# hidasib/GRU4Rec

Measured on AMD Instinct MI355X. Metric: mini-batches/sec (gru4rec.py:661), RSC15-shaped batch=128 n_sample=2048 BPR-max, higher is better.
Workload: dtype f32

## Files before the change

gru4rec_amd/csrc/g4r_device.cuh:

```cuda
#pragma once
#include <hip/hip_runtime.h>
#include <stdint.h>

#include "../../include/gru4rec_hip.h"

typedef float f32x4 __attribute__((ext_vector_type(4)));

#define G4R_EPS_LOSS 1e-24f
#define G4R_EPS_ADAGRAD 1e-6f

#if defined(G4R_MUTATE) && G4R_MUTATE == 1
#define G4R_MUT_ACC(x) ((x) * 1.01f)
#else
#define G4R_MUT_ACC(x) (x)
#endif
#if defined(G4R_MUTATE) && G4R_MUTATE == 2
#define G4R_MUT_STEP(x) ((x) * 1.01f)
#else
#define G4R_MUT_STEP(x) (x)
#endif
#if defined(G4R_MUTATE) && G4R_MUTATE == 3
#define G4R_MUT_DACC(x) ((x) * 1.01f)
#else
#define G4R_MUT_DACC(x) (x)
#endif

#if defined(G4R_MUTATE) && G4R_MUTATE == 6
#define G4R_MUT_ROW(n, x) ((n) == 0 ? (x) * 1.5f : (x))
#else
#define G4R_MUT_ROW(n, x) (x)
#endif
#if defined(G4R_MUTATE) && G4R_MUTATE == 5
#define G4R_MUT_XSCALE(x) ((x) * 1.01f)
#else
#define G4R_MUT_XSCALE(x) (x)
#endif

#define G4R_STREAM_SAMPLE 0x53414D50u
#define G4R_STREAM_DROP_EMBED 0x44454D42u
#define G4R_STREAM_DROP_HIDDEN 0x44484944u
#define G4R_STREAM_TIEBREAK 0x54494542u

#if defined(__HIP_DEVICE_COMPILE__)
#define GAS __attribute__((address_space(1)))
#else
#define GAS
#endif
#define GP(T) GAS T*

__device__ __forceinline__ float4 ld4(const GAS float* p) { return *(const GAS float4*)p; }
__device__ __forceinline__ void st4(GAS float* p, float4 v) { *(GAS float4*)p = v; }
__device__ __forceinline__ int4 ldi4(const GAS int* p) { return *(const GAS int4*)p; }
#if defined(__HIP_DEVICE_COMPILE__)
// ... 60 lines not shown
    GP(const int) in_idx; GP(const int) out_idx; GP(const int) Mplan;
    GP(const unsigned char) reset;
    GP(const int) ST;
    int gl;
    GP(const float) lq_tgt; GP(const float) lq_smp;
    GP(StepState) st;
    GP(long long) dbgclk;
    GP(const float) zrow;
    GP(long long) dbgtile;
    GP(float) xbase;
    long long xstride;
    int xn, xoffSx, xoffSy, xoffSBy;
    int xmode, xoffDg;
    GP(float) dyp;
    int bbn[G4R_MAX_LAYERS];
    GP(float) vp;
    int defer_mask, dRcap;
    long long dSx_stride, dSy_stride, dSBy_stride;
    GP(int) last_use;
    GP(int) dcand;
    GP(int) dlist;
    GP(unsigned) dstat;
    GP(float) drp;
};
#define G4R_SLOT(m, g) ((size_t)((g) & (long long)(m).defer_mask))
#define G4R_DSX(m, g) ((m).dSx + G4R_SLOT(m, g) * (size_t)(m).dSx_stride)
#define G4R_DSY(m, g) ((m).dSy + G4R_SLOT(m, g) * (size_t)(m).dSy_stride)
#define G4R_DSBY(m, g) ((m).dSBy + G4R_SLOT(m, g) * (size_t)(m).dSBy_stride)

#if defined(G4R_CLK_TRACE)
#define G4R_DBGCLK(m) ((m).dbgclk)
#define G4R_DBGTILE(m) ((m).dbgtile)
#else
#define G4R_DBGCLK(m) ((GAS long long*)nullptr)
#define G4R_DBGTILE(m) ((GAS long long*)nullptr)
#endif
#define G4R_TICK(m, kern, phase)                                                                     \
    do {                                                                                             \
        if (G4R_DBGCLK(m) && blockIdx.x == 0 && blockIdx.y == 0 && threadIdx.x == 0)                  \
            G4R_DBGCLK(m)[(kern) * 16 + (phase)] = wall_clock64();                                       \
    } while (0)

template <int CTRL>
__device__ __forceinline__ float dpp_mov(float v) {
    return __builtin_bit_cast(float, __builtin_amdgcn_update_dpp(0, __builtin_bit_cast(int, v), CTRL, 0xF, 0xF, true));
}
// ... 138 lines not shown
```

gru4rec_amd/csrc/g4r_host_create.hpp:

```cpp

int g4r_device_count(void) {
    int n = 0;
    if (hipGetDeviceCount(&n) != hipSuccess) return 0;
    return n;
}
const char* g4r_last_error(void) { return g_err.c_str(); }
#ifndef G4R_HIPCC_VERSION
#define G4R_HIPCC_VERSION "unknown"
#endif
const char* g4r_version(void) { return "gru4rec_hip 0.4 (gfx950; hipcc " G4R_HIPCC_VERSION "; isa-audited)"; }
int g4r_sizeof_config(void) { return (int)sizeof(g4r_config); }

static int build_lean_args(g4r_model* m) {
    DevModel& d = m->dm;
    const StepKernels& k = m->kern;
    const int L = d.n_layers;
    std::vector<LeanV> av(L); std::vector<LeanH> ah(L); std::vector<LeanDa> aa(L); std::vector<LeanDy> ay(L);
    const bool constrained = d.embed_mode == G4R_EMBED_CONSTRAINED;
    bool any_layer = false;
    for (int l = 0; l < L; ++l) {
        if (k.fwd[l] != FWD_LEAN) continue;
        any_layer = true;
        LeanV& v = av[l]; memset(&v, 0, sizeof(v));
        v.Wx = d.dense_p + d.offWx[l]; v.Wrz = d.dense_p + d.offWrz[l]; v.Bh = d.dense_p + d.offBh[l];
// ... 33 lines not shown
        q.col_item = d.col_item; q.occ_idx = d.occ_idx + d.B; q.occ_fl = d.occ_fl; q.mp = nullptr; q.dbg = d.dbgclk; q.dbgtile = d.dbgtile; q.R = d.R; q.pub_fl = d.xmode == 0 ? 1 : 0; q.logq = d.logq;
        m->h_leanS = q;
        if (dalloc(m, &m->d_leanS, (size_t)1)) return -1;
    }
    if (k.score_bwd == SB_LEAN) {
        LeanB q; memset(&q, 0, sizeof(q));
        q.accBy = d.accBy; q.occ_fl = d.occ_fl; q.dSy = d.dSy; q.dAy = d.dAy; q.dSBy = d.dSBy; q.dABy = d.dABy; q.dhpart = d.dhpart; q.dbg = d.dbgclk; q.dbgtile = d.dbgtile;
        q.dSy_stride = d.dSy_stride; q.dSBy_stride = d.dSBy_stride; q.defer_mask = d.defer_mask; q.generic = d.generic;
        q.ndh = cdiv(d.Dtop + 1, 64); q.nA = cdiv(d.ldSc, 16) * q.ndh; q.nrb = cdiv(d.B, 16); q.ndb = cdiv(d.Dtop, 64); q.lr = d.lr;
        m->h_leanB = q;
        if (dalloc(m, &m->d_leanB, (size_t)1)) return -1;
        HIPCHK(hipMemcpyAsync(m->d_leanB, &m->h_leanB, sizeof(LeanB), hipMemcpyHostToDevice, m->stream));
    }
    if (k.update == UP_LEAN) {
        LeanU u; memset(&u, 0, sizeof(u));
        u.mp = nullptr; u.st = d.st; u.Wy = d.Wy; u.E = d.E; u.accWy = d.accWy; u.accE = d.accE; u.velWy = d.velWy; u.velE = d.velE;
        u.By = d.By; u.accBy = d.accBy; u.velBy = d.velBy; u.dAx = d.dAx; u.dAy = d.dAy; u.dABy = d.dABy;
        u.dense_p = d.dense_p; u.dense_acc = d.dense_acc; u.dense_vel = d.dense_vel; u.yin0 = d.yin0; u.meta = d.cur_in + 2 * d.B;
        u.dbg = d.dbgclk; u.dbgtile = d.dbgtile; u.n_items = d.n_items; u.constrained = constrained ? 1 : 0; u.wE = d.Ein; u.wY = d.Dtop;
        u.lr = d.lr; u.mom = d.mom; u.lmbd = d.lmbd;
        m->h_leanU = u;
        const std::vector<DenseTile> tiles = dense_tiles(d, 16, 64);
        m->ntiles16 = (int)tiles.size();
        if (dalloc(m, &m->d_tiles16, tiles.size()) || dalloc(m, &m->d_leanU, (size_t)1)) return -1;
        HIPCHK(hipMemcpyAsync(m->d_tiles16, tiles.data(), tiles.size() * sizeof(DenseTile), hipMemcpyHostToDevice, m->stream));
        HIPCHK(hipStreamSynchronize(m->stream));
    }
    HIPCHK(hipStreamSynchronize(m->stream));
    return 0;
}

static KernelSwitches read_switches(const g4r_config& cfg) {
    KernelSwitches w;
    w.no_lean = getenv("G4R_NO_LEAN") != nullptr; w.no_mt = getenv("G4R_NO_MT") != nullptr; w.no_bmt = getenv("G4R_NO_BMT") != nullptr;
    w.no_merge = getenv("G4R_NO_MERGE") != nullptr;
    w.allow_lean_update = env_int("G4R_LEAN_UPDATE", 1) != 0; w.defer = env_int("G4R_DEFER", cfg.defer_updates) != 0;
    w.p2_geo = env_int("G4R_P2_GEO", -1); w.ba_geo = env_int("G4R_BA_GEO", -1);
    w.wide2 = env_int("G4R_WIDE2", -1); w.p1_ks = env_int("G4R_P1_KS", 128); w.bb_ks = env_int("G4R_BB_KS", 0);
    const char* skip = getenv("G4R_SKIP_KN");
    w.skip_kn = skip ? strtoull(skip, nullptr, 0) : 0ull;
    return w;
}

int g4r_create(const g4r_config* cfg, g4r_model** out) {
    if (!cfg || !out) return fail("null argument");
    if (cfg->n_layers < 1 || cfg->n_layers > G4R_MAX_LAYERS) return fail("n_layers out of range");
    if (cfg->batch_size < 1 || cfg->n_items < 1) return fail("batch_size / n_items must be positive");
    for (int l = 0; l < cfg->n_layers; ++l)
        if (cfg->layers[l] % 4 != 0 || cfg->layers[l] < 4 || cfg->layers[l] > 1024)
            return fail("layer sizes must be multiples of 4 in [4, 1024]");
    if (cfg->embed_mode == G4R_EMBED_SEPARATE && (cfg->embedding % 4 != 0 || cfg->embedding < 4 || cfg->embedding > 1024))
        return fail("embedding must be a multiple of 4 in [4, 1024]");
    if (cfg->embed_mode != G4R_EMBED_CONSTRAINED && cfg->embed_mode != G4R_EMBED_SEPARATE && cfg->embed_mode != G4R_EMBED_ONEHOT)
        return fail("unsupported embedding mode");
    if (cfg->embed_mode == G4R_EMBED_ONEHOT && 3 * cfg->layers[0] > 1024)
        return fail("one-hot input: 3 * layers[0] must be <= 1024 (row width of the Wx[0] table)");
    if (cfg->loss < 0 || cfg->loss > G4R_LOSS_XE_LOGIT) return fail("unsupported loss");
    if (cfg->smoothing != 0.f && cfg->loss != G4R_LOSS_XE && cfg->loss != G4R_LOSS_XE_LOGIT) return fail("smoothing needs a cross-entropy loss");
// ... 251 lines not shown
```

gru4rec_amd/csrc/g4r_host_debug.hpp:

```cpp
int g4r_get_debug(g4r_model* m, const char* name, float* host, int64_t count) {
    if (!m || !name || !host) return fail("null argument");
    HIPCHK(hipSetDevice(m->cfg.device));
    DevModel& d = m->dm;
    const StepKernels& k = m->kern;
    std::string s(name);
    const float* p = nullptr; int64_t n = 0;
    int l = 0;
    if (!s.empty() && isdigit((unsigned char)s.back())) { l = s.back() - '0'; s.pop_back(); }
    if (l >= d.n_layers) return fail("layer out of range");
    const int64_t bd = (int64_t)d.B * d.D[l];
    if (s == "scores") { p = d.Sc; n = (int64_t)d.B * d.ldSc; }
    else if (s == "dSx") { p = d.dSx + (size_t)((m->gstep - 1) & d.defer_mask) * (size_t)d.dSx_stride; n = (int64_t)d.B * d.Ein; }
    else if (s == "dSy") { p = d.dSy + (size_t)((m->gstep - 1) & d.defer_mask) * (size_t)d.dSy_stride; n = (int64_t)d.ldSc * d.Dtop; }
    else if (s == "dSBy") { p = d.dSBy + (size_t)((m->gstep - 1) & d.defer_mask) * (size_t)d.dSBy_stride; n = d.ldSc; }
    else if (s == "defer_stats") {
        if (count < 4) return fail("count");
        double rows = 0, bias = 0;
        if (m->defer_on) {
            std::vector<unsigned> st(2048);
            HIPCHK(hipStreamSynchronize(m->stream));
            HIPCHK(hipMemcpy(st.data(), d.dstat, st.size() * sizeof(unsigned), hipMemcpyDeviceToHost));
            for (size_t i = 0; i < st.size(); i += 2) { rows += st[i]; bias += st[i + 1]; }
        }
        host[0] = (float)rows; host[1] = (float)bias; host[2] = m->defer_on ? 1.f : 0.f; host[3] = (float)(d.defer_mask + 1);
        return 0;
    }
    else if (s == "dhpart") { p = d.dhpart; n = (int64_t)d.ksplit * d.B * d.Dtop; }
    else if (s == "lossrow") { p = d.lossrow; n = d.B; }
    else if (s == "hd") { p = d.hd[l]; n = bd; }
    else if (s == "r") { p = d.r[l]; n = bd; }
    else if (s == "z") { p = d.z[l]; n = bd; }
    else if (s == "c") { p = d.c[l]; n = bd; }
    else if (s == "Hr") { p = d.Hr[l]; n = bd; }
    else if (s == "dV") { p = d.dV[l]; n = bd * 3; }
    else if (s == "dyl") { p = d.dyl[l]; n = bd; }
    else if (s == "Hprev") { p = d.H[l][(m->gstep + 1) & 1]; n = bd; }
    else if (s == "occ_idx") { p = (const float*)d.occ_idx; n = d.R; }
#if !defined(G4R_CLK_TRACE)
    else if (s == "dbgclk" || s == "dbgtile") return fail("in-kernel traces need a library built with G4R_BUILD_CLK=1 (python -m gru4rec_amd.build --force) and G4R_CLK=1 at run time");
#endif
    else if (s == "dbgclk") { if (!d.dbgclk) return fail("G4R_CLK not set"); p = (const float*)d.dbgclk; n = 2 * (64 + 8 * (int64_t)d.R); }
    else if (s == "dbgtile") { if (!d.dbgtile) return fail("G4R_CLK not set"); p = (const float*)d.dbgtile; n = 2 * 8 * (int64_t)8192; }
    else if (s == "ntiles") { if (count < 1) return fail("count"); host[0] = (float)m->ntiles; return 0; }
    else if (s == "ldSc") { if (count < 1) return fail("count"); host[0] = (float)d.ldSc; return 0; }
    else if (s == "wide_mask") {
        if (count < 1) return fail("count");
        int mk = k.wide_dense ? 16 : 0;
        for (int l = 0; l < d.n_layers; ++l) mk |= k.wg[l].use;
        host[0] = (float)mk; return 0;
    }
    else if (s == "deep_geo") {
        if (count < 1) return fail("count");
        host[0] = (float)(k.p2_deep[0] + 2 * k.ba_deep[0]); return 0;
    }
    else if (s == "score_mt") { if (count < 1) return fail("count"); host[0] = k.score_fwd == SF_MT ? 272.f : 0.f; return 0; }
    else if (s == "score_bmt") { if (count < 1) return fail("count"); host[0] = (float)k.bmt_slabs; return 0; }
    else if (s == "lean") {
        if (count < 4) return fail("count");
        int mk = 0;
        for (int l = 0; l < d.n_layers; ++l) mk |= k.fwd[l] == FWD_LEAN ? 1 << l : 0;
// ... 161 lines not shown
```

gru4rec_amd/csrc/g4r_host_model.hpp:

```cpp
static thread_local std::string g_err;
static int fail(const std::string& s) { g_err = s; return -1; }
void g4r_set_error(const char* fmt, ...) {
    char buf[1024];
    va_list ap;
    va_start(ap, fmt);
    vsnprintf(buf, sizeof(buf), fmt, ap);
    va_end(ap);
    g_err = buf;
}
#define HIPCHK(x)                                                                                        \
    do {                                                                                                 \
        hipError_t e_ = (x);                                                                             \
        if (e_ != hipSuccess)                                                                            \
            return fail(std::string(#x) + ": " + hipGetErrorString(e_) + " @" + std::to_string(__LINE__)); \
    } while (0)
#define NCCLCHK(x)                                                                                         \
    do {                                                                                                   \
        ncclResult_t e_ = (x);                                                                             \
        if (e_ != ncclSuccess)                                                                             \
            return fail(std::string(#x) + ": " + ncclGetErrorString(e_) + " @" + std::to_string(__LINE__)); \
    } while (0)

enum { KN_GRU_P1 = 0, KN_GRU_P2, KN_SCORE_FWD, KN_LOSS, KN_SCORE_BWD, KN_BWD_PRE, KN_BWD_A, KN_BWD_B, KN_DENSE, KN_ALLREDUCE,
       KN_DENSE_APPLY, KN_SPARSE, KN_UPDATE, KN_BWD_FUSED, KN_FWD_FUSED, KN_GATE, KN_FLUSH, KN_SCAN, KN_FINISH, KN_GRU_V, KN_GRU_H, KN_GRU_DA, KN_GRU_DY, KN_COUNT };
static const char* KN_NAMES[KN_COUNT] = {"k_gru_p1", "k_gru_p2", "k_score_fwd", "k_loss_rows", "k_score_bwd", "k_gru_bwd_pre",
                                         "k_gru_bwd_a", "k_gru_bwd_b", "k_dense_grad", "rccl_allreduce", "k_dense_apply",
                                         "k_sparse_update", "k_update", "k_gru_bwd", "k_gru_fwd", "k_gru_gate", "k_sparse_flush", "k_defer_scan", "k_finish_rows", "k_gru_v", "k_gru_h", "k_gru_da", "k_gru_dy"};

struct EvRec { int kn; hipEvent_t a, b; };

struct KernelSwitches {
    bool no_lean = false;
    bool no_mt = false, no_bmt = false;
    bool no_merge = false;
    bool allow_lean_update = true;
    bool defer = false;
    int p2_geo = -1, ba_geo = -1;
    int wide2 = -1, p1_ks = 128, bb_ks = 0;
    unsigned long long skip_kn = 0;
};
enum GruFwdKind { FWD_LEAN = 0 , FWD_FUSED = 1 , FWD_P1S = 2 ,
                  FWD_P1_N64 = 3, FWD_P1_N32 = 4 };
enum GruBwdKind { BWD_LEAN = 0 , BWD_FUSED = 1 , BWD_ONEHOT = 2, BWD_BW = 3, BWD_B = 4 };
enum ScoreFwdKind { SF_LEAN = 0 , SF_MT = 1 , SF_T3 = 2, SF_T2 = 3, SF_K64 = 4, SF_K128 = 5  };
enum ScoreBwdKind { SB_LEAN = 0 , SB_BMT = 1 , SB_BWD2 = 2 , SB_W = 3, SB_N = 4  };
enum UpdateKind { UP_LEAN = 0 , UP_MERGED = 1 , UP_SPLIT = 2 };
struct WideGeo { int use = 0, ny = 1, nh = 1, kys = 0, khs = 0, bbn = 1, bbk = 0; };
struct StepKernels {
    int fwd[G4R_MAX_LAYERS], bwd[G4R_MAX_LAYERS];
    int p2_deep[G4R_MAX_LAYERS], ba_deep[G4R_MAX_LAYERS];
    WideGeo wg[G4R_MAX_LAYERS];
    int score_fwd;
    int loss_spec, loss_long, loss_quads;
    int score_bwd;
    int kch, ksplit;
    int bmt_slabs;
    int nblkA, nblkB, ndtA, ndtB, nrtB;
    int update;
// ... 287 lines not shown
```

gru4rec_amd/csrc/g4r_host_step.hpp:

```cpp
static int launch_step(g4r_model* m, std::vector<EvRec>* recs, int part = 0) {
    DevModel& d = m->dm;
    const StepKernels& k = m->kern;
    const int L = d.n_layers, B = d.B;
    hipStream_t s = m->stream;
    GruFwdPredict nopa = {};
    size_t evi = 0;
    hipEvent_t cur_a = nullptr, cur_b = nullptr;
    static const bool trace = getenv("G4R_TRACE") != nullptr;
    int trace_kn = -1;
    auto begin = [&](int kn) {
        trace_kn = kn;
        if (trace) { fprintf(stderr, "[g4r] launch %s\n", KN_NAMES[kn]); fflush(stderr); }
        if (!recs) return;
        while (m->evs.size() < evi + 2) { hipEvent_t e; (void)hipEventCreate(&e); m->evs.push_back(e); }
        EvRec r = {kn, m->evs[evi], m->evs[evi + 1]};
        evi += 2;
        cur_a = r.a; cur_b = r.b;
        recs->push_back(r);
    };
    auto end = [&]() {
        if (trace) {
            hipError_t e = hipStreamSynchronize(s);
            fprintf(stderr, "[g4r] done   %s: %s\n", KN_NAMES[trace_kn], hipGetErrorString(e));
            fflush(stderr);
// ... 58 lines not shown
    }
    begin(KN_SCORE_FWD);
    switch (k.score_fwd) {
    case SF_LEAN: {
        const unsigned dimsA = (unsigned)d.Dtop | ((unsigned)B << 16), dimsB = (unsigned)d.N | ((unsigned)d.ldSc << 16);
        const dim3 gs(cdiv(d.ldSc, 32), cdiv(B, 32));
        if (d.logq != 0.f) LK(k_score_s<true>, gs, dim3(256), 0, s, (const LeanS*)m->d_leanS, (const int*)(d.cur_in + 2 * B), (const int*)d.cur_col, (const float*)d.hd[L - 1],
                              (const float*)d.Wy, (const float*)d.By, (float*)d.Sc, dimsA, dimsB);
        else LK(k_score_s<false>, gs, dim3(256), 0, s, (const LeanS*)m->d_leanS, (const int*)(d.cur_in + 2 * B), (const int*)d.cur_col, (const float*)d.hd[L - 1],
                (const float*)d.Wy, (const float*)d.By, (float*)d.Sc, dimsA, dimsB);
        break;
    }
    case SF_MT: LK(k_score_mt_4s, dim3(cdiv(B, 64) * cdiv(d.ldSc, 272)), dim3(256), SMEM_MT_4S, s, (const int*)d.cur_col, (const int*)(d.cur_in + 2 * B),
                   (const float*)d.hd[L - 1], (const float*)d.Wy, (const float*)d.zrow, dmp, (unsigned)d.Dtop | ((unsigned)cdiv(B, 64) << 16),
                   (unsigned)d.N, (unsigned)d.ldSc, (unsigned)B); break;
    case SF_T3: LK(k_score_fwd_t3, dim3(cdiv(d.ldSc, 64), cdiv(B, 64)), dim3(GT_NTH), SMEM_SF3, s, dmp, stp); break;
    case SF_T2: LK(k_score_fwd_t2, dim3(cdiv(d.ldSc, 64), cdiv(B, 64)), dim3(GT_NTH), SMEM_SF2, s, dmp, stp); break;
    case SF_K64: LK(k_score_fwd_k64, dim3(cdiv(d.ldSc, SFW_BN), cdiv(B, SF_BM)), dim3(GT_NTH), SMEM_SF64, s, dmp, stp); break;
    default: LK(k_score_fwd_k128, dim3(cdiv(d.ldSc, GT_BN), cdiv(B, SF_BM)), dim3(GT_NTH), SMEM_SF, s, dmp, stp); break;
    }
    end();
    begin(KN_LOSS);
    {
#define G4R_LK_LOSS(L, V)                                                                                                      \
        do {                                                                                                                   \
            if (k.loss_spec == 1) LK((k_loss_rows<L, 1, V>), dim3(B), dim3(LOSS_T), m->smem_loss, s, dmp, stp);      \
            else if (k.loss_spec == 2) LK((k_loss_rows<L, 2, V>), dim3(B), dim3(LOSS_T), m->smem_loss, s, dmp, stp); \
            else if (k.loss_spec == 3) LK((k_loss_rows<L, 3, V>), dim3(B), dim3(LOSS_T), m->smem_loss, s, dmp, stp); \
            else LK((k_loss_rows<L, 0, V>), dim3(B), dim3(LOSS_T), m->smem_loss, s, dmp, stp);                       \
        } while (0)
        if (k.loss_long) G4R_LK_LOSS(true, 4);
        else { if (k.loss_quads) G4R_LK_LOSS(false, 4); else G4R_LK_LOSS(false, 1); }
#undef G4R_LK_LOSS
    }
    end();
    begin(KN_SCORE_BWD);
    switch (k.score_bwd) {
    case SB_LEAN: {
        const LeanB& q = m->h_leanB;
        LK(k_score_b, dim3(q.nA + d.ksplit * q.nrb * q.ndb), dim3(512), 0, s, (const LeanB*)m->d_leanB, (const int*)(d.cur_in + 2 * B), (const int*)d.cur_col,
           (const float*)d.Sc, (const float*)d.hd[L - 1], (const float*)d.Wy, (float*)d.accWy, (unsigned)d.Dtop | ((unsigned)B << 16), (unsigned)d.N | ((unsigned)d.ldSc << 16));
        break;
    }
    case SB_BMT: {
        const int ntile = d.ldSc / BMT_WA * (d.Dtop / 32);
        LK(k_score_bmt, dim3(2 * ntile), dim3(256), SMEM_BMT, s, (const float*)d.Sc, (const float*)d.hd[L - 1], (const float*)d.Wy, (const int*)d.col_item,
           (const int*)(d.cur_in + 2 * B), (const float*)d.zrow, dmp, (unsigned)d.Dtop | ((unsigned)(d.Dtop / 32) << 16), (unsigned)d.N | ((unsigned)d.ldSc << 16),
           (unsigned)B | ((unsigned)d.kch << 16), (unsigned)cdiv(B, 64) | ((unsigned)(d.Dtop / 128) << 16));
        break;
    }
    case SB_BWD2: {
        const int ndt = d.Dtop / 64, nrt = cdiv(B, 64);
// ... 474 lines not shown
```

gru4rec_amd/csrc/g4r_lean_kernels.cuh:

```cuda
#pragma once

#define LN_MAXD 128

__device__ __forceinline__ float ldu(const GAS float* base, unsigned boff) { return *(const GAS float*)((const GAS char*)base + boff); }
__device__ __forceinline__ int ldu_i(const GAS int* base, unsigned boff) { return *(const GAS int*)((const GAS char*)base + boff); }
__device__ __forceinline__ float4 ldu4(const GAS float* base, unsigned boff) { return *(const GAS float4*)((const GAS char*)base + boff); }
__device__ __forceinline__ void stu(GAS float* base, unsigned boff, float v) { *(GAS float*)((GAS char*)base + boff) = v; }
__device__ __forceinline__ void stu4(GAS float* base, unsigned boff, float4 v) { *(GAS float4*)((GAS char*)base + boff) = v; }

#if defined(G4R_CLK_TRACE)
#define LCLK_INIT(dbgp, slot) GAS long long* clk_ = ((dbgp) && blockIdx.x == 1 && blockIdx.y == 1 && blockIdx.z == 0 && threadIdx.x == 0) ? (dbgp) + (slot) : nullptr
#define LCLK(i) do { if (clk_) clk_[i] = wall_clock64(); } while (0)
#define LCLK_USE(x) do { if (clk_ && (x) == 123.456f) clk_[15] = 0; } while (0)
#define LSPAN_BEGIN(tilep, base) GAS long long* span_ = ((tilep) && threadIdx.x == 0) ? (tilep) + 8 * (size_t)((base) + (blockIdx.z * gridDim.y + blockIdx.y) * gridDim.x + blockIdx.x) : nullptr; \
    if (span_) span_[0] = wall_clock64()
#define LSPAN_END() do { if (span_) span_[1] = wall_clock64(); } while (0)
#else
#define LCLK_INIT(dbgp, slot)
#define LCLK(i)
#define LCLK_USE(x)
#define LSPAN_BEGIN(tilep, base)
#define LSPAN_END()
#endif

// ... 49 lines not shown
    GP(long long) dbg; GP(long long) dbgtile;
    int R, pub_fl;
    float logq, pad;
};

struct LeanB {
    GP(float) accBy; GP(const int) occ_fl; GP(float) dSy; GP(float) dAy; GP(float) dSBy; GP(float) dABy; GP(float) dhpart;
    GP(long long) dbg; GP(long long) dbgtile;
    long long dSy_stride, dSBy_stride;
    int defer_mask, generic, nA, ndh, nrb, ndb;
    float lr, pad;
};

struct LeanU {
    const DevModel* mp; StepState* st;
    GP(float) Wy; GP(float) E; GP(float) accWy; GP(float) accE; GP(float) velWy; GP(float) velE;
    GP(float) By; GP(float) accBy; GP(float) velBy;
    GP(const float) dAx; GP(const float) dAy; GP(const float) dABy;
    GP(float) dense_p; GP(float) dense_acc; GP(float) dense_vel; GP(const float) yin0;
    GP(const int) meta;
    GP(long long) dbg; GP(long long) dbgtile;
    int n_items, constrained, wE, wY;
    float lr, mom, lmbd, pad;
};

template <typename T> __device__ __forceinline__ void lean_pin1(T v) {
#if defined(__HIP_DEVICE_COMPILE__)
    asm volatile("" ::"s"(v));
#endif
}
template <typename... T> __device__ __forceinline__ void lean_pin(T... v) { (lean_pin1(v), ...); }
__device__ __forceinline__ void lean_keep(float& x) {
#if defined(__HIP_DEVICE_COMPILE__)
    asm volatile("" : "+v"(x));
#endif
}
struct LeanState { unsigned g; int M; unsigned t_lo; };
__device__ __forceinline__ LeanState lean_state(int4 mt) {
    LeanState s;
    s.g = (unsigned)__builtin_amdgcn_readfirstlane(mt.x); s.M = __builtin_amdgcn_readfirstlane(mt.z); s.t_lo = (unsigned)__builtin_amdgcn_readfirstlane(mt.w);
    return s;
}

template <bool L0, bool DROPE>
__global__ __launch_bounds__(512) void k_gru_v(const LeanV* __restrict__ ap, StepState* st_, const int* cur_in_, const float* Wx_, const float* Wrz_,
                                               const float* H0_, const float* H1_, unsigned dims, unsigned B) {
// ... 597 lines not shown
#pragma unroll
        for (int u = 0; u < 4; ++u) {
            const bool kok = nk + u < ldSc && nk == nkc && its[u] >= 0 && dq < D;
            const float av_ = bok ? dsx[u] : 0.f;
            const float4 w4 = kok ? wv[u] : make_float4(0.f, 0.f, 0.f, 0.f);
            acc[0] = mfma16(av_, w4.x, acc[0]);
            acc[1] = mfma16(av_, w4.y, acc[1]);
            acc[2] = mfma16(av_, w4.z, acc[2]);
            acc[3] = mfma16(av_, w4.w, acc[3]);
        }
#pragma unroll
        for (int rg = 0; rg < 4; ++rg) sJ[(rg * 8 + wid) * 64 + lane] = (f32x4){acc[0][rg], acc[1][rg], acc[2][rg], acc[3][rg]};
        __syncthreads();
        if (wid >= 4) return;
        f32x4 v = sJ[(wid * 8 + 0) * 64 + lane];
#pragma unroll
        for (int w = 1; w < 8; ++w) v += sJ[(wid * 8 + w) * 64 + lane];
        const unsigned b = b0 + 4 * lg + (wid & 3);
        if ((int)b < M && dq < D) st4(a.dhpart + ((size_t)kc * B + b) * D + dq, make_float4(v[0], v[1], v[2], v[3]));
        LSPAN_END();
    }
}

#if defined(G4R_MUTATE) && G4R_MUTATE == 8
#define G4R_MUT_SLICE_SKIP(j, base0, start) ((base0) > (start) && (j) == (base0) + 1023)
#else
#define G4R_MUT_SLICE_SKIP(j, base0, start) false
#endif
template <bool MOM>
__device__ __forceinline__ void lean_rows_update(const LeanU& a, const GAS int* occ_idx, GAS int* occ_fl, const GAS float* dSx, const GAS float* dSy,
                                                 const GAS float* dSBy, unsigned k, unsigned R, unsigned B) {
    const unsigned lane = threadIdx.x & 63;
    const bool tableE = k < B && !a.constrained;
    const unsigned W = tableE ? (unsigned)a.wE : (unsigned)a.wY, nc4 = W >> 2;
    const unsigned c4 = min(lane, nc4 - 1);
    const bool lok = lane < nc4;
    const unsigned kc = min(k, R - 1);
    int item = ldu_i(occ_idx, 4 * kc);
    const GAS float* srow = (kc < B) ? dSx + (size_t)kc * W : dSy + (size_t)(kc - B) * W;
    const float4 sk = ld4(srow + 4 * c4);
    const bool bias = k >= B;
    const float bsk = bias ? dSBy[kc - B] : 0.f;
    lean_pin(a.Wy, a.E, a.accWy, a.accE, a.By, a.accBy, a.dAx, a.dAy, a.dABy, a.n_items, a.lr, a.mom, a.lmbd);
    if (k >= R) item = -1;
    GAS float* P = tableE ? a.E : a.Wy;
    GAS float* A = tableE ? a.accE : a.accWy;
    GAS float* V = tableE ? a.velE : a.velWy;
    const unsigned ic = (unsigned)max(item, 0);
    GAS int* flp = occ_fl + 4 * ((tableE ? (size_t)a.n_items : 0) + ic);
    const int4 fl = ldi4(flp);
    const float4 pz = ld4(P + (size_t)ic * W + 4 * c4);
    float4 vz = make_float4(0.f, 0.f, 0.f, 0.f);
    if (MOM) vz = ld4(V + (size_t)ic * W + 4 * c4);
    const float bpz = a.By[ic];
    float bvz = 0.f;
    if (MOM) bvz = a.velBy[ic];
    const bool owner = item >= 0 && fl.x == (int)k + 1;
    if (!owner) return;
    if (lane == 0) *(GAS int4*)flp = make_int4(0, 0, 0, 0);
    const float lr = a.lr, momc = a.mom, lmbd = a.lmbd;
    const int n = fl.z;
    const int lo = (a.constrained || k < B) ? 0 : (int)B;
    const int first_j = max(lo, (int)R - fl.y);
    float4 S = make_float4(0.f, 0.f, 0.f, 0.f);
    float Sb = 0.f;
    int nb_e = 0;
    if (n > 1) {
        if (first_j >= 2 * (int)B) {
            for (int cdup = 1; cdup < n; ++cdup) { S.x += sk.x; S.y += sk.y; S.z += sk.z; S.w += sk.w; Sb += bsk; }
            nb_e = n - 1;
        } else {
            for (int base0 = first_j & ~3; base0 < (int)k; base0 += 1024) {
                int4 vv[4];
#pragma unroll
                for (int u = 0; u < 4; ++u) vv[u] = ldi4(occ_idx + min(base0 + 256 * u + 4 * (int)lane, (int)((R + 3) & ~3u) - 4));
#pragma unroll
                for (int u = 0; u < 4; ++u) {
                    const int j0 = base0 + 256 * u + 4 * (int)lane;
                    const int ids[4] = {vv[u].x, vv[u].y, vv[u].z, vv[u].w};
                    unsigned long long mk[4];
#pragma unroll
                    for (int e = 0; e < 4; ++e) mk[e] = __ballot(ids[e] == item && j0 + e >= first_j && j0 + e < (int)k && !G4R_MUT_SLICE_SKIP(j0 + e, base0, first_j & ~3));
                    unsigned long long any = mk[0] | mk[1] | mk[2] | mk[3];
                    while (any) {
                        int js[8], nj = 0;
                        while (any && nj < 8) {
                            const int l = __builtin_ctzll(any);
                            bool more = false;
#pragma unroll
                            for (int e = 0; e < 4; ++e) {
                                if ((mk[e] >> l) & 1ull) {
                                    if (nj < 8) {
                                        const int jv = base0 + 256 * u + 4 * l + e;
// ... 25 lines not shown
                }
            }
        }
    }
    const float fn = (float)n;
    const float p0[4] = {pz.x, pz.y, pz.z, pz.w}, v0[4] = {vz.x, vz.y, vz.z, vz.w}, sl[4] = {sk.x, sk.y, sk.z, sk.w};
    const float ss[4] = {S.x + sk.x, S.y + sk.y, S.z + sk.z, S.w + sk.w};
    float pn[4], vn[4];
#pragma unroll
    for (int e = 0; e < 4; ++e) {
        const float reg = (lmbd > 0.f) ? lr * lmbd * p0[e] : 0.f;
        const float tot = (lmbd > 0.f) ? ss[e] + fn * reg : ss[e];
        if (MOM) { vn[e] = momc * v0[e] - (sl[e] + reg); pn[e] = p0[e] + (fn * (momc * v0[e]) - tot); }
        else { vn[e] = 0.f; pn[e] = p0[e] - tot; }
    }
    float bn = 0.f, bvn = 0.f;
    if (bias) {
        const float fb = (float)(nb_e + 1);
        const float reg = (lmbd > 0.f) ? lr * lmbd * bpz : 0.f;
        const float sb = Sb + bsk;
        const float tot = (lmbd > 0.f) ? sb + fb * reg : sb;
        if (MOM) { bn = bpz + (fb * (momc * bvz) - tot); bvn = momc * bvz - (bsk + reg); }
        else bn = bpz - tot;
    }
    float4 ak = make_float4(0.f, 0.f, 0.f, 0.f);
    float bak = 0.f;
    if (n > 1) {
        const GAS float* arow = (k < B) ? a.dAx + (size_t)k * W : a.dAy + (size_t)(k - B) * W;
        ak = ld4(arow + 4 * c4);
        if (bias) bak = a.dABy[k - B];
    }
    lean_keep(bn); lean_keep(bvn); lean_keep(bak);
    const size_t o = (size_t)item * W + 4 * c4;
    if (lok) {
        st4(P + o, make_float4(pn[0], pn[1], pn[2], pn[3]));
        if (MOM) st4(V + o, make_float4(vn[0], vn[1], vn[2], vn[3]));
        if (n > 1) st4(A + o, ak);
    }
    if (bias && lane == 0) {
        a.By[item] = bn;
        if (MOM) a.velBy[item] = bvn;
        if (n > 1) a.accBy[item] = bak;
    }
}

template <bool MOM>
__device__ __forceinline__ void lean_dense_tile(const LeanU& a, const DenseTile* tiles_, unsigned tile, unsigned B) {
    __shared__ f32x4 sJ[4 * 8 * 64];
    const unsigned tid = threadIdx.x, lane = tid & 63, li = lane & 15, lg = lane >> 4;
    const unsigned wid = __builtin_amdgcn_readfirstlane(tid >> 6);
    const GAS DenseTile* tiles = (const GAS DenseTile*)tiles_;
    const DenseTile tl = tiles[tile];
    const GAS StepState* sg = (const GAS StepState*)a.st;
// ... 90 lines not shown
        } else if (tid - 64 < B) {
            const unsigned b = tid - 64;
            ci[b] = in_idx[t1 * B + b];
            ci[B + b] = reset[t1 * B + b];
        }
        return;
    }
    const int n = 512 * (int)(part - 1) + (int)tid;
    const int vo = out_idx[t1 * B + min(n, (int)B - 1)];
    const int vs = (ns > 0) ? ST[(size_t)(gl > 0 ? g1 % gl : 0) * ns + min(max(n - (int)B, 0), ns - 1)] : -1;
    if (n < ld) cc[n] = (n < Mn) ? vo : (n >= (int)B && n < N && Mn > 0) ? vs : -1;
}

template <bool MOM>
__global__ __launch_bounds__(512) void k_update_l(const LeanU* __restrict__ ap, const DenseTile* __restrict__ tiles_, const int* occ_idx_, int* occ_fl_,
                                                  const float* dSx_, const float* dSy_, const float* dSBy_, unsigned packA, unsigned packB, unsigned nbk) {
    const unsigned ntiles = packA & 0xFFFFu, nblk = packA >> 16, R = packB & 0xFFFFu, B = packB >> 16;
    const LeanU a = *ap;
    LSPAN_BEGIN(a.dbgtile, 2700);
    if (blockIdx.x < nbk) { lean_bookkeep(a, blockIdx.x, B); LSPAN_END(); return; }
    const unsigned b = blockIdx.x - nbk;
    if (b < ntiles) { lean_dense_tile<MOM>(a, tiles_, b, B); LSPAN_END(); return; }
    const unsigned q = b - ntiles, wid = __builtin_amdgcn_readfirstlane(threadIdx.x >> 6);
    lean_rows_update<MOM>(a, (const GAS int*)occ_idx_, (GAS int*)occ_fl_, (const GAS float*)dSx_, (const GAS float*)dSy_, (const GAS float*)dSBy_, wid * nblk + q, R, B);
    LSPAN_END();
}
template __global__ void k_update_l<false>(const LeanU*, const DenseTile*, const int*, int*, const float*, const float*, const float*, unsigned, unsigned, unsigned);
template __global__ void k_update_l<true>(const LeanU*, const DenseTile*, const int*, int*, const float*, const float*, const float*, unsigned, unsigned, unsigned);
```

gru4rec_amd/csrc/g4r_loss_kernel.cuh:

```cuda
#pragma once
#ifndef LOSS_T
#define LOSS_T 1024
#endif
#define LOSS_NW (LOSS_T / 64)
template <int NV, bool MAX>
__device__ __forceinline__ void block_reduce(float (&v)[NV], float* red) {
    const int lane = threadIdx.x & 63, w = threadIdx.x >> 6;
#pragma unroll
    for (int q = 0; q < NV; ++q) v[q] = MAX ? wave_max(v[q]) : wave_sum(v[q]);
    if (lane == 0) {
#pragma unroll
        for (int q = 0; q < NV; ++q) red[q * LOSS_NW + w] = v[q];
    }
    __syncthreads();
#pragma unroll
    for (int q = 0; q < NV; ++q) {
        float a = red[q * LOSS_NW];
#pragma unroll
        for (int u = 1; u < LOSS_NW; ++u) a = MAX ? fmaxf(a, red[q * LOSS_NW + u]) : a + red[q * LOSS_NW + u];
        v[q] = a;
    }
}

__device__ __forceinline__ float softplusf_(float x) {
    return fmaxf(x, 0.f) + log1pf(fexp(-fabsf(x)));
}

template <int V, class Ptr>
__device__ __forceinline__ void vld(float (&o)[V], Ptr p) {
    if constexpr (V == 4) { const float4 t = ld4(p); o[0] = t.x; o[1] = t.y; o[2] = t.z; o[3] = t.w; }
    else o[0] = p[0];
}
template <int V, class Ptr>
__device__ __forceinline__ void vst(Ptr p, const float (&o)[V]) {
    if constexpr (V == 4) st4(p, make_float4(o[0], o[1], o[2], o[3]));
    else p[0] = o[0];
}

template <bool LONG_ROW, int SPEC, int V>
__global__ __launch_bounds__(LOSS_T) void k_loss_rows(const DevModel* __restrict__ mp, StepState* st) {
    const DevModel& m = *mp;
    extern __shared__ __attribute__((aligned(16))) float smem[];
    const int tid = threadIdx.x;
    const int B = m.B, N = m.N, i = blockIdx.x;
    const int fact = SPEC == 1 || SPEC == 3 ? (int)G4R_ACT_ELU : (SPEC == 2 ? (int)G4R_ACT_SOFTMAX : m.final_act);
    const int lossk = SPEC == 1 ? (int)G4R_LOSS_BPR_MAX : (SPEC == 2 ? (int)G4R_LOSS_XE : (SPEC == 3 ? (int)G4R_LOSS_TOP1_MAX : m.loss));
    const int ldSc = m.ldSc;
    const float fp0 = m.fa_p0, fp1 = m.fa_p1, invB = m.inv_B, bpreg = m.bpreg, smooth = m.smoothing;
    GAS float* row = m.Sc + (size_t)i * ldSc;
    float* sy = smem;
    std::conditional_t<LONG_ROW, GAS float*, float*> se;
    if constexpr (LONG_ROW) se = row; else se = smem + ldSc;
    float* red = smem + (LONG_ROW ? 1 : 2) * ldSc;
    constexpr int STEP = V * LOSS_T;
    const int jt = V * tid;
    constexpr int LOSS_PRE = (V == 4) ? 2 : 4;
    const StepCtx c = load_ctx(st);
    float pre_s[LOSS_PRE][V];
#pragma unroll
    for (int q = 0; q < LOSS_PRE; ++q) vld<V>(pre_s[q], row + min(jt + q * STEP, ldSc - V));
    const int M = c.M;
    if (i >= M) return;
    const bool fsm = (fact == G4R_ACT_SOFTMAX), fsl = (fact == G4R_ACT_SOFTMAX_LOGIT);
    const float n_out = (float)(M + (N - B));
    auto active = [&](int j) { return j < N && (j < M || j >= B); };
    auto grp_fast = [&](int j0) { return (j0 >= B && j0 + V <= N) || (j0 + V <= M && (i < j0 || i >= j0 + V)); };
    using Fast = std::true_type;
    using Slow = std::false_type;
#define G4R_GROUPS(lim, fn) for (int j0 = jt; j0 < (lim); j0 += STEP) { if (grp_fast(j0)) fn(Fast{}, j0); else fn(Slow{}, j0); }
    float mneg[1] = {0.f};
    if (fsm || fsl) {
        float mx[1] = {-INFINITY};
        auto first = [&](auto F, int j0, const float (&v)[V]) {
            float o[V];
#pragma unroll
            for (int e = 0; e < V; ++e) {
                const bool a = F.value || active(j0 + e);
                o[e] = a ? v[e] : 0.f;
                mx[0] = a ? fmaxf(mx[0], v[e]) : mx[0];
            }
// ... 268 lines not shown
```

Measured before the change: 24730.

## Precompute duplicate-occurrence positions in spare loss-kernel blocks for sparse update

Extra blocks are added to the loss kernel launch. They prescan the occurrence index for each owner row with duplicates and record up to 15 earlier positions in a small table appended to the tiles buffer. The sparse row update then reads these positions and gathers those gradient rows directly, instead of scanning the whole occurrence list itself. The dAx/dAy load is also hoisted before the accumulation. This moves the serial scan off the update kernel's critical path and overlaps it with the loss work, at the cost of extra loss-kernel blocks and some extra memory traffic.

```diff
diff --git a/gru4rec_amd/csrc/g4r_device.cuh b/gru4rec_amd/csrc/g4r_device.cuh
--- a/gru4rec_amd/csrc/g4r_device.cuh
+++ b/gru4rec_amd/csrc/g4r_device.cuh
@@ -8,6 +8,7 @@
 
 #define G4R_EPS_LOSS 1e-24f
 #define G4R_EPS_ADAGRAD 1e-6f
+#define G4R_OWN_INLINE 15
 
 #if defined(G4R_MUTATE) && G4R_MUTATE == 1
 #define G4R_MUT_ACC(x) ((x) * 1.01f)
@@ -29,6 +30,11 @@
 #define G4R_MUT_ROW(n, x) ((n) == 0 ? (x) * 1.5f : (x))
 #else
 #define G4R_MUT_ROW(n, x) (x)
+#endif
+#if defined(G4R_MUTATE) && G4R_MUTATE == 8
+#define G4R_MUT_SLICE_SKIP(j, base0, start) ((base0) > (start) && (j) == (base0) + 1023)
+#else
+#define G4R_MUT_SLICE_SKIP(j, base0, start) false
 #endif
 #if defined(G4R_MUTATE) && G4R_MUTATE == 5
 #define G4R_MUT_XSCALE(x) ((x) * 1.01f)
@@ -135,6 +141,7 @@
     GP(int) dlist;
     GP(unsigned) dstat;
     GP(float) drp;
+    GP(int) own_pos;
 };
 #define G4R_SLOT(m, g) ((size_t)((g) & (long long)(m).defer_mask))
 #define G4R_DSX(m, g) ((m).dSx + G4R_SLOT(m, g) * (size_t)(m).dSx_stride)
diff --git a/gru4rec_amd/csrc/g4r_host_create.hpp b/gru4rec_amd/csrc/g4r_host_create.hpp
--- a/gru4rec_amd/csrc/g4r_host_create.hpp
+++ b/gru4rec_amd/csrc/g4r_host_create.hpp
@@ -79,7 +79,10 @@
         m->h_leanU = u;
         const std::vector<DenseTile> tiles = dense_tiles(d, 16, 64);
         m->ntiles16 = (int)tiles.size();
-        if (dalloc(m, &m->d_tiles16, tiles.size()) || dalloc(m, &m->d_leanU, (size_t)1)) return -1;
+        const size_t nslot = cdiv((long long)d.R * 16 * sizeof(int), (long long)sizeof(DenseTile));
+        if (dalloc(m, &m->d_tiles16, tiles.size() + nslot) || dalloc(m, &m->d_leanU, (size_t)1)) return -1;
+        d.own_pos = m->sw.owner_scan_in_update ? nullptr : (int*)(m->d_tiles16 + tiles.size());
+        m->h_leanU.own_on = d.own_pos ? 1 : 0;
         HIPCHK(hipMemcpyAsync(m->d_tiles16, tiles.data(), tiles.size() * sizeof(DenseTile), hipMemcpyHostToDevice, m->stream));
         HIPCHK(hipStreamSynchronize(m->stream));
     }
@@ -90,7 +93,7 @@
 static KernelSwitches read_switches(const g4r_config& cfg) {
     KernelSwitches w;
     w.no_lean = getenv("G4R_NO_LEAN") != nullptr; w.no_mt = getenv("G4R_NO_MT") != nullptr; w.no_bmt = getenv("G4R_NO_BMT") != nullptr;
-    w.no_merge = getenv("G4R_NO_MERGE") != nullptr;
+    w.no_merge = getenv("G4R_NO_MERGE") != nullptr; w.owner_scan_in_update = env_int("G4R_OWNER_SCAN", 0) != 0;
     w.allow_lean_update = env_int("G4R_LEAN_UPDATE", 1) != 0; w.defer = env_int("G4R_DEFER", cfg.defer_updates) != 0;
     w.p2_geo = env_int("G4R_P2_GEO", -1); w.ba_geo = env_int("G4R_BA_GEO", -1);
     w.wide2 = env_int("G4R_WIDE2", -1); w.p1_ks = env_int("G4R_P1_KS", 128); w.bb_ks = env_int("G4R_BB_KS", 0);
diff --git a/gru4rec_amd/csrc/g4r_host_debug.hpp b/gru4rec_amd/csrc/g4r_host_debug.hpp
--- a/gru4rec_amd/csrc/g4r_host_debug.hpp
+++ b/gru4rec_amd/csrc/g4r_host_debug.hpp
@@ -36,6 +36,7 @@
     else if (s == "dyl") { p = d.dyl[l]; n = bd; }
     else if (s == "Hprev") { p = d.H[l][(m->gstep + 1) & 1]; n = bd; }
     else if (s == "occ_idx") { p = (const float*)d.occ_idx; n = d.R; }
+    else if (s == "own_pos") { if (!d.own_pos) return fail("no owner table (k_update_l not chosen, or G4R_OWNER_SCAN=1)"); p = (const float*)d.own_pos; n = 16 * (int64_t)d.R; }
 #if !defined(G4R_CLK_TRACE)
     else if (s == "dbgclk" || s == "dbgtile") return fail("in-kernel traces need a library built with G4R_BUILD_CLK=1 (python -m gru4rec_amd.build --force) and G4R_CLK=1 at run time");
 #endif
diff --git a/gru4rec_amd/csrc/g4r_host_model.hpp b/gru4rec_amd/csrc/g4r_host_model.hpp
--- a/gru4rec_amd/csrc/g4r_host_model.hpp
+++ b/gru4rec_amd/csrc/g4r_host_model.hpp
@@ -34,6 +34,7 @@
     bool no_mt = false, no_bmt = false;
     bool no_merge = false;
     bool allow_lean_update = true;
+    bool owner_scan_in_update = false;
     bool defer = false;
     int p2_geo = -1, ba_geo = -1;
     int wide2 = -1, p1_ks = 128, bb_ks = 0;
diff --git a/gru4rec_amd/csrc/g4r_host_step.hpp b/gru4rec_amd/csrc/g4r_host_step.hpp
--- a/gru4rec_amd/csrc/g4r_host_step.hpp
+++ b/gru4rec_amd/csrc/g4r_host_step.hpp
@@ -104,12 +104,14 @@
     end();
     begin(KN_LOSS);
     {
+        const int nown = std::min(cdiv(d.R, LOSS_NW), std::max(2 * m->n_cu - B, 32));
+        const dim3 gloss(B + (merged && k.update == UP_LEAN && d.own_pos ? nown : 0));
 #define G4R_LK_LOSS(L, V)                                                                                                      \
         do {                                                                                                                   \
-            if (k.loss_spec == 1) LK((k_loss_rows<L, 1, V>), dim3(B), dim3(LOSS_T), m->smem_loss, s, dmp, stp);      \
-            else if (k.loss_spec == 2) LK((k_loss_rows<L, 2, V>), dim3(B), dim3(LOSS_T), m->smem_loss, s, dmp, stp); \
-            else if (k.loss_spec == 3) LK((k_loss_rows<L, 3, V>), dim3(B), dim3(LOSS_T), m->smem_loss, s, dmp, stp); \
-            else LK((k_loss_rows<L, 0, V>), dim3(B), dim3(LOSS_T), m->smem_loss, s, dmp, stp);                       \
+            if (k.loss_spec == 1) LK((k_loss_rows<L, 1, V>), gloss, dim3(LOSS_T), m->smem_loss, s, dmp, stp);        \
+            else if (k.loss_spec == 2) LK((k_loss_rows<L, 2, V>), gloss, dim3(LOSS_T), m->smem_loss, s, dmp, stp);   \
+            else if (k.loss_spec == 3) LK((k_loss_rows<L, 3, V>), gloss, dim3(LOSS_T), m->smem_loss, s, dmp, stp);   \
+            else LK((k_loss_rows<L, 0, V>), gloss, dim3(LOSS_T), m->smem_loss, s, dmp, stp);                         \
         } while (0)
         if (k.loss_long) G4R_LK_LOSS(true, 4);
         else { if (k.loss_quads) G4R_LK_LOSS(false, 4); else G4R_LK_LOSS(false, 1); }
diff --git a/gru4rec_amd/csrc/g4r_lean_kernels.cuh b/gru4rec_amd/csrc/g4r_lean_kernels.cuh
--- a/gru4rec_amd/csrc/g4r_lean_kernels.cuh
+++ b/gru4rec_amd/csrc/g4r_lean_kernels.cuh
@@ -95,6 +95,7 @@
     GP(long long) dbg; GP(long long) dbgtile;
     int n_items, constrained, wE, wY;
     float lr, mom, lmbd, pad;
+    int own_on, pad2;
 };
 
 template <typename T> __device__ __forceinline__ void lean_pin1(T v) {
@@ -738,14 +739,9 @@
     }
 }
 
-#if defined(G4R_MUTATE) && G4R_MUTATE == 8
-#define G4R_MUT_SLICE_SKIP(j, base0, start) ((base0) > (start) && (j) == (base0) + 1023)
-#else
-#define G4R_MUT_SLICE_SKIP(j, base0, start) false
-#endif
 template <bool MOM>
 __device__ __forceinline__ void lean_rows_update(const LeanU& a, const GAS int* occ_idx, GAS int* occ_fl, const GAS float* dSx, const GAS float* dSy,
-                                                 const GAS float* dSBy, unsigned k, unsigned R, unsigned B) {
+                                                 const GAS float* dSBy, const GAS int* opos_t, unsigned k, unsigned R, unsigned B) {
     const unsigned lane = threadIdx.x & 63;
     const bool tableE = k < B && !a.constrained;
     const unsigned W = tableE ? (unsigned)a.wE : (unsigned)a.wY, nc4 = W >> 2;
@@ -753,6 +749,7 @@
     const bool lok = lane < nc4;
     const unsigned kc = min(k, R - 1);
     int item = ldu_i(occ_idx, 4 * kc);
+    const int opos = ldu_i(opos_t, 4 * (16 * kc + min(lane, 15u)));
     const GAS float* srow = (kc < B) ? dSx + (size_t)kc * W : dSy + (size_t)(kc - B) * W;
     const float4 sk = ld4(srow + 4 * c4);
     const bool bias = k >= B;
@@ -773,9 +770,16 @@
     if (MOM) bvz = a.velBy[ic];
     const bool owner = item >= 0 && fl.x == (int)k + 1;
     if (!owner) return;
+    const int n = fl.z;
+    float4 ak = make_float4(0.f, 0.f, 0.f, 0.f);
+    float bak = 0.f;
+    if (n > 1) {
+        const GAS float* arow = (k < B) ? a.dAx + (size_t)k * W : a.dAy + (size_t)(k - B) * W;
+        ak = ld4(arow + 4 * c4);
+        if (bias) bak = a.dABy[k - B];
+    }
     if (lane == 0) *(GAS int4*)flp = make_int4(0, 0, 0, 0);
     const float lr = a.lr, momc = a.mom, lmbd = a.lmbd;
-    const int n = fl.z;
     const int lo = (a.constrained || k < B) ? 0 : (int)B;
     const int first_j = max(lo, (int)R - fl.y);
     float4 S = make_float4(0.f, 0.f, 0.f, 0.f);
@@ -785,6 +789,30 @@
         if (first_j >= 2 * (int)B) {
             for (int cdup = 1; cdup < n; ++cdup) { S.x += sk.x; S.y += sk.y; S.z += sk.z; S.w += sk.w; Sb += bsk; }
             nb_e = n - 1;
+        } else if (a.own_on && __builtin_amdgcn_readfirstlane(opos) >= 0) {
+            const int ln = __builtin_amdgcn_readfirstlane(opos);
+            for (int q0 = 0; q0 < ln; q0 += 8) {
+                const int nj = min(8, ln - q0);
+                int js[8];
+#pragma unroll
+                for (int q = 0; q < 8; ++q) js[q] = __builtin_amdgcn_readlane(opos, 1 + min(q0 + q, ln - 1));
+                float4 g[8];
+                float gb[8];
+#pragma unroll
+                for (int q = 0; q < 8; ++q) {
+                    const int jj = js[q];
+                    const GAS float* r2 = (jj < (int)B) ? dSx + (size_t)jj * W : dSy + (size_t)(jj - (int)B) * W;
+                    g[q] = ld4(r2 + 4 * c4);
+                    gb[q] = (bias && jj >= (int)B) ? dSBy[jj - (int)B] : 0.f;
+                }
+#pragma unroll
+                for (int q = 0; q < 8; ++q) {
+                    if (q < nj) {
+                        S.x += g[q].x; S.y += g[q].y; S.z += g[q].z; S.w += g[q].w;
+                        if (js[q] >= (int)B) { Sb += gb[q]; ++nb_e; }
+                    }
+                }
+            }
         } else {
             for (int base0 = first_j & ~3; base0 < (int)k; base0 += 1024) {
                 int4 vv[4];
@@ -856,13 +884,6 @@
         const float tot = (lmbd > 0.f) ? sb + fb * reg : sb;
         if (MOM) { bn = bpz + (fb * (momc * bvz) - tot); bvn = momc * bvz - (bsk + reg); }
         else bn = bpz - tot;
-    }
-    float4 ak = make_float4(0.f, 0.f, 0.f, 0.f);
-    float bak = 0.f;
-    if (n > 1) {
-        const GAS float* arow = (k < B) ? a.dAx + (size_t)k * W : a.dAy + (size_t)(k - B) * W;
-        ak = ld4(arow + 4 * c4);
-        if (bias) bak = a.dABy[k - B];
     }
     lean_keep(bn); lean_keep(bvn); lean_keep(bak);
     const size_t o = (size_t)item * W + 4 * c4;
@@ -999,7 +1020,8 @@
     const unsigned b = blockIdx.x - nbk;
     if (b < ntiles) { lean_dense_tile<MOM>(a, tiles_, b, B); LSPAN_END(); return; }
     const unsigned q = b - ntiles, wid = __builtin_amdgcn_readfirstlane(threadIdx.x >> 6);
-    lean_rows_update<MOM>(a, (const GAS int*)occ_idx_, (GAS int*)occ_fl_, (const GAS float*)dSx_, (const GAS float*)dSy_, (const GAS float*)dSBy_, wid * nblk + q, R, B);
+    lean_rows_update<MOM>(a, (const GAS int*)occ_idx_, (GAS int*)occ_fl_, (const GAS float*)dSx_, (const GAS float*)dSy_, (const GAS float*)dSBy_,
+                          (const GAS int*)(tiles_ + ntiles), wid * nblk + q, R, B);
     LSPAN_END();
 }
 template __global__ void k_update_l<false>(const LeanU*, const DenseTile*, const int*, int*, const float*, const float*, const float*, unsigned, unsigned, unsigned);
diff --git a/gru4rec_amd/csrc/g4r_loss_kernel.cuh b/gru4rec_amd/csrc/g4r_loss_kernel.cuh
--- a/gru4rec_amd/csrc/g4r_loss_kernel.cuh
+++ b/gru4rec_amd/csrc/g4r_loss_kernel.cuh
@@ -35,6 +35,55 @@
 __device__ __forceinline__ void vst(Ptr p, const float (&o)[V]) {
     if constexpr (V == 4) st4(p, make_float4(o[0], o[1], o[2], o[3]));
     else p[0] = o[0];
+}
+
+__device__ __forceinline__ void owner_prescan(const DevModel& m, unsigned k) {
+    const unsigned lane = threadIdx.x & 63;
+    const unsigned R = (unsigned)m.R, B = (unsigned)m.B;
+    const GAS int* occ_idx = m.occ_idx;
+    int item = occ_idx[min(k, R - 1)];
+    if (k >= R) item = -1;
+    if (item < 0) return;
+    const bool constrained = m.embed_mode == G4R_EMBED_CONSTRAINED;
+    const bool tableE = k < B && !constrained;
+    const int4 fl = ldi4(m.occ_fl + 4 * ((tableE ? (size_t)m.n_items : 0) + (unsigned)item));
+    if (fl.x != (int)k + 1 || fl.z < 2) return;
+    const int lo = (constrained || k < B) ? 0 : (int)B;
+    const int first_j = max(lo, (int)R - fl.y);
+    if (first_j >= 2 * (int)B) return;
+    GAS int* pos = m.own_pos + 16 * (size_t)k;
+    if (fl.z - 1 > G4R_OWN_INLINE) {
+        if (lane == 0) pos[0] = -1;
+        return;
+    }
+    const unsigned long long below = (1ull << lane) - 1ull;
+    int cnt = 0;
+    for (int base0 = first_j & ~3; base0 < (int)k; base0 += 1024) {
+        int4 vv[4];
+#pragma unroll
+        for (int u = 0; u < 4; ++u) vv[u] = ldi4(occ_idx + min(base0 + 256 * u + 4 * (int)lane, (int)((R + 3) & ~3u) - 4));
+#pragma unroll
+        for (int u = 0; u < 4; ++u) {
+            const int j0 = base0 + 256 * u + 4 * (int)lane;
+            const int ids[4] = {vv[u].x, vv[u].y, vv[u].z, vv[u].w};
+            unsigned long long mk[4];
+            int at = cnt;
+#pragma unroll
+            for (int e = 0; e < 4; ++e) {
+                mk[e] = __ballot(ids[e] == item && j0 + e >= first_j && j0 + e < (int)k && !G4R_MUT_SLICE_SKIP(j0 + e, base0, first_j & ~3));
+                at += __popcll(mk[e] & below);
+                cnt += __popcll(mk[e]);
+            }
+#pragma unroll
+            for (int e = 0; e < 4; ++e) {
+                if ((mk[e] >> lane) & 1ull) {
+                    if ((unsigned)at < (unsigned)G4R_OWN_INLINE) pos[1 + at] = j0 + e;
+                    ++at;
+                }
+            }
+        }
+    }
+    if (lane == 0) pos[0] = min(cnt, G4R_OWN_INLINE);
 }
 
 template <bool LONG_ROW, int SPEC, int V>
@@ -55,7 +104,16 @@
     constexpr int STEP = V * LOSS_T;
     const int jt = V * tid;
     constexpr int LOSS_PRE = (V == 4) ? 2 : 4;
+#if defined(G4R_CLK_TRACE)
+    struct Span { GAS long long* p; __device__ ~Span() { if (p) p[1] = wall_clock64(); } } span_{(m.dbgtile && tid == 0 && i < 1024) ? m.dbgtile + 8 * (size_t)(7168 + i) : nullptr};
+    if (span_.p) span_.p[0] = wall_clock64();
+#endif
     const StepCtx c = load_ctx(st);
+    if (i >= B) {
+        const unsigned nown = gridDim.x - B, R = m.R;
+        for (unsigned k = (threadIdx.x >> 6) * nown + (unsigned)(i - B); k < R; k += LOSS_NW * nown) owner_prescan(m, k);
+        return;
+    }
     float pre_s[LOSS_PRE][V];
 #pragma unroll
     for (int q = 0; q < LOSS_PRE; ++q) vld<V>(pre_s[q], row + min(jt + q * STEP, ldSc - V));
```

Measured after the change: 25790, median of 6. 4.3% higher.
